# HKUST-Aerial-Robotics/FUEL

Measured on AMD Instinct MI355X. Metric: plan_cycles_per_sec, higher is better.
Workload: dtype u64 bit-planes / u16 (u32 beyond 255 voxels) exact squared distances / f32 ESDF / f64 log-odds and B-spline

## Files before the change

### fuel_amd/csrc/esdf.hip

```cpp
#include <algorithm>
#include <cmath>
#include <vector>

#include "fuelmi_internal.h"

template <int MODE>
__device__ __forceinline__ u64 src_word(const u64* __restrict__ infl, const u64* __restrict__ unk, long w) {
  if (MODE == 0) return infl[w] | unk[w];
  if (MODE == 1) return infl[w];
  return ~infl[w];
}

template <int MODE>
__device__ __forceinline__ int nearest_src(const u64* __restrict__ infl, const u64* __restrict__ unk,
                                           long linebit, int zlo, int zhi, int z) {
  int best = -1;
  {
    long pos = linebit + z, end = linebit + zhi;
    long w = pos >> 6;
    u64 word = src_word<MODE>(infl, unk, w) & (~0ull << (pos & 63));
    while (true) {
      if (word) {
        long c = (w << 6) + __builtin_ctzll(word);
        if (c <= end) best = (int)(c - pos);
// ... 516 lines not shown
  int below, above;
};
template <int NW>
struct LineBits {
  u64 w[NW];
};
template <int MODE, int NW>
__device__ __forceinline__ LineBits<NW> line_load(const u64* __restrict__ infl, const u64* __restrict__ unk, long linebit,
                                                  int z0a, int zlo, int zhi) {
  const long bit0 = linebit + z0a;
  const long w0 = bit0 >> 6;
  const int sh = (int)(bit0 & 63);
  u64 L[NW + 1];
#pragma unroll
  for (int k = 0; k <= NW; ++k) L[k] = src_word<MODE>(infl, unk, w0 + k);
  LineBits<NW> r;
#pragma unroll
  for (int k = 0; k < NW; ++k) {
    const int lo = max(zlo - z0a - 64 * k, 0), hi = min(zhi - z0a - 64 * k, 63);
    const u64 mask = lo <= hi ? bit_range(lo, hi - lo + 1) : 0ull;
    r.w[k] = (sh ? ((L[k] >> sh) | (L[k + 1] << (64 - sh))) : L[k]) & mask;
  }
  return r;
}
template <int NW>
__device__ __forceinline__ u32 line_bits32(const LineBits<NW>& L, int s) {
  const int k = s >> 6, sh = s & 63;
  u64 lo = 0ull, hi = 0ull;
#pragma unroll
  for (int i = 0; i < NW; ++i) {
    if (i == k) lo = L.w[i];
    if (i == k + 1) hi = L.w[i];
  }
  return (u32)(sh ? ((lo >> sh) | (hi << (64 - sh))) : lo);
}
template <int NW>
__device__ __forceinline__ int line_first_from(const LineBits<NW>& L, int s) {
  int pos = -1;
#pragma unroll
  for (int i = NW - 1; i >= 0; --i) {
    u64 m = L.w[i];
    if (64 * i + 63 < s)
      m = 0ull;
    else if (64 * i < s)
      m &= ~0ull << (s - 64 * i);
    if (m) pos = 64 * i + __builtin_ctzll(m);
  }
  return pos;
}
template <int NW>
__device__ __forceinline__ int line_last_below(const LineBits<NW>& L, int s) {
  int pos = -1;
#pragma unroll
  for (int i = 0; i < NW; ++i) {
    u64 m = L.w[i];
    if (64 * i >= s)
      m = 0ull;
    else if (64 * i + 64 > s)
      m &= (1ull << (s - 64 * i)) - 1ull;
    if (m) pos = 64 * i + 63 - __builtin_clzll(m);
  }
  return pos;
}
template <int NW, bool BELOW>
__device__ __forceinline__ RowSrc row_src_line(const LineBits<NW>& L, int z0a, int zc0, int ZC) {
  RowSrc r;
  const int s = zc0 - z0a;
  r.bits = (u64)(line_bits32<NW>(L, s) & (ZC == 32 ? 0xffffffffu : ((1u << ZC) - 1u)));
  const int up = line_first_from<NW>(L, s + ZC);
  r.above = up >= 0 ? z0a + up : -1;
  r.below = -1;
  if (BELOW) {
    const int dn = line_last_below<NW>(L, s);
    r.below = dn >= 0 ? z0a + dn : -1;
  }
  return r;
}

__device__ __forceinline__ u32 bit_fill(u32 v, int zi) {
  u32 r;
  asm("v_bfe_i32 %0, %1, %2, 1" : "=v"(r) : "v"(v), "s"(zi));
  return r;
}
template <int G>
__device__ __forceinline__ u32 zy_fill_pair(u32* prow, u32 bA, u32 bB, u32 d0, int aboveA, int aboveB, int ze, u32 inbox, bool fast) {
  constexpr int ZC = 4 * G;
  const u32 full = ZC == 32 ? 0xffffffffu : ((1u << (ZC & 31)) - 1u);
  if (fast) {
    const bool all_src = bA == inbox && bB == inbox && inbox != 0u;
    const bool no_src = (bA | bB) == 0u && d0 == 0x00ff00ffu && aboveA < 0 && aboveB < 0;
    if (__ballot(!(all_src | no_src)) == 0ull) {
      const u32 v = all_src ? 0u : pk_both(PK_INF);
      const uint4 o = make_uint4(v, v, v, v);
#pragma unroll
      for (int k = 0; k < G; ++k) *reinterpret_cast<uint4*>(prow + 4 * k) = o;
      if (inbox != full) {
        const u32 ib = inbox | (threadIdx.x & 0u);
        for (int zi = 0; zi < ZC; ++zi) prow[zi] &= bit_fill(ib, zi);
      }
      return all_src ? 0u : 0x00ff00ffu;
    }
  }
  const u32 nA = ~bA, nB = ~bB;
  u32 nm[ZC];
  u32 d = d0;
#pragma unroll
  for (int k = 0; k < G; ++k) {
    u32 f[4];
#pragma unroll
    for (int q = 0; q < 4; ++q) {
      const int zi = 4 * k + q;
      nm[zi] = (bit_fill(nA, zi) & 0xffffu) | (bit_fill(nB, zi) & 0xffff0000u);
      d = pk_add(d, 0x00010001u) & nm[zi];
      f[q] = d;
    }
    *reinterpret_cast<uint4*>(prow + 4 * k) = make_uint4(f[0], f[1], f[2], f[3]);
  }
  const u32 d_end = pk_min(d, 0x00ff00ffu);
  d = (aboveA >= 0 ? (u32)min(aboveA - (ze + 1), 255) : 255u) | ((aboveB >= 0 ? (u32)min(aboveB - (ze + 1), 255) : 255u) << 16);
#pragma unroll
  for (int k = G - 1; k >= 0; --k) {
    const uint4 fw = *reinterpret_cast<const uint4*>(prow + 4 * k);
    const u32 f[4] = {fw.x, fw.y, fw.z, fw.w};
    u32 o[4];
#pragma unroll
    for (int q = 3; q >= 0; --q) {
      d = pk_add(d, 0x00010001u) & nm[4 * k + q];
      const u32 t = pk_min(pk_min(f[q], d), 0x00ff00ffu);
      o[q] = pk_mul(t, t);
    }
    *reinterpret_cast<uint4*>(prow + 4 * k) = make_uint4(o[0], o[1], o[2], o[3]);
  }
  if (inbox != full) {
    const u32 ib = inbox | (threadIdx.x & 0u);
    for (int zi = 0; zi < ZC; ++zi) prow[zi] &= bit_fill(ib, zi);
  }
  return d_end;
}
__device__ __forceinline__ u32 pk_below_d0(const RowSrc& A, const RowSrc& B, int zs) {
  return (A.below >= 0 ? (u32)min(zs - 1 - A.below, 255) : 255u) | ((B.below >= 0 ? (u32)min(zs - 1 - B.below, 255) : 255u) << 16);
}

__device__ __noinline__ u32 pk_slow_col(const u32* tile, int ZC, int ylen, int row, int zcol) {
  u32 best = INF32;
  const int rmax = max(row, ylen - 1 - row);
  for (int r = 0; r <= rmax && (u32)(r * r) < best; ++r) {
    const u32 rr = (u32)(r * r);
    if (row - r >= 0) {
      const int q = row - r;
      const u32 v = (tile[(q >> 1) * ZC + zcol] >> (16 * (q & 1))) & 0xffffu;
      if (v < PK_INF) best = min(best, v + rr);
    }
    if (r && row + r < ylen) {
      const int q = row + r;
      const u32 v = (tile[(q >> 1) * ZC + zcol] >> (16 * (q & 1))) & 0xffffu;
      if (v < PK_INF) best = min(best, v + rr);
    }
  }
  return best;
}

template <int G, bool TILE_SLOW = true>
__device__ __forceinline__ void pk_scan8(const unsigned char* tile_b, int p, int gi, int npair, int ylen, bool any_src,
                                         bool sampled, int& n_far, uint4& ra, uint4& rb) {
  constexpr int ZC = 4 * G;
  constexpr int stride = ZC * 4;
  const u32* tile = reinterpret_cast<const u32*>(tile_b);
    const int col = 16 * gi, base = __mul24(p, stride) + col;
    if (!any_src) {
      ra = rb = make_uint4(INF32, INF32, INF32, INF32);
      if (sampled) n_far += __popcll(__ballot(1));
    } else {
      const uint4 v = lds4(tile_b, base);
      u32 b0 = pk_min(v.x, pk_adds(pk_swap(v.x), 0x00010001u)), b1 = pk_min(v.y, pk_adds(pk_swap(v.y), 0x00010001u));
      u32 b2 = pk_min(v.z, pk_adds(pk_swap(v.z), 0x00010001u)), b3 = pk_min(v.w, pk_adds(pk_swap(v.w), 0x00010001u));
      u32 mx = pk_hmax(pk_max(pk_max(b0, b1), pk_max(b2, b3)));
      const int hi_off = __mul24(npair - 1, stride) + col;
      const int jmax = max(p, npair - 1 - p);
      int od = base, ou = base;
      u32 ro2 = 1u, j8 = 8u;
      for (int j = 1; j <= jmax && ro2 < mx; ++j) {
        od = max(od - stride, col);
        ou = min(ou + stride, hi_off);
        const uint4 pd = lds4(tile_b, od), pu = lds4(tile_b, ou);
        const u32 rn2 = ro2 + j8;
        const u32 re2 = (ro2 + rn2 - 2u) >> 1;
        const u32 ke = pk_both(pk_sat16(re2));
        const u32 k1 = pk_sat16(ro2) | (pk_sat16(rn2) << 16), k2 = pk_sat16(rn2) | (pk_sat16(ro2) << 16);
        b0 = pk_min(b0, pk_min(pk_adds(pk_min(pd.x, pu.x), ke), pk_min(pk_adds(pk_swap(pd.x), k1), pk_adds(pk_swap(pu.x), k2))));
        b1 = pk_min(b1, pk_min(pk_adds(pk_min(pd.y, pu.y), ke), pk_min(pk_adds(pk_swap(pd.y), k1), pk_adds(pk_swap(pu.y), k2))));
        b2 = pk_min(b2, pk_min(pk_adds(pk_min(pd.z, pu.z), ke), pk_min(pk_adds(pk_swap(pd.z), k1), pk_adds(pk_swap(pu.z), k2))));
        b3 = pk_min(b3, pk_min(pk_adds(pk_min(pd.w, pu.w), ke), pk_min(pk_adds(pk_swap(pd.w), k1), pk_adds(pk_swap(pu.w), k2))));
        mx = pk_hmax(pk_max(pk_max(b0, b1), pk_max(b2, b3)));
        ro2 = rn2;
        j8 += 8u;
      }
      if (sampled) n_far += __popcll(__ballot(pk_hmin(pk_min(pk_min(b0, b1), pk_min(b2, b3))) > ESDF_FAR_D * ESDF_FAR_D));
      ra = make_uint4(b0 & 0xffffu, b1 & 0xffffu, b2 & 0xffffu, b3 & 0xffffu);
      rb = make_uint4(b0 >> 16, b1 >> 16, b2 >> 16, b3 >> 16);
      if (TILE_SLOW && mx >= PK_INF) {
        const int zc = 4 * gi, rA = 2 * p, rB = 2 * p + 1;
        if (ra.x >= PK_INF) ra.x = pk_slow_col(tile, ZC, ylen, rA, zc);
        if (ra.y >= PK_INF) ra.y = pk_slow_col(tile, ZC, ylen, rA, zc + 1);
        if (ra.z >= PK_INF) ra.z = pk_slow_col(tile, ZC, ylen, rA, zc + 2);
        if (ra.w >= PK_INF) ra.w = pk_slow_col(tile, ZC, ylen, rA, zc + 3);
        if (rB < ylen) {
          if (rb.x >= PK_INF) rb.x = pk_slow_col(tile, ZC, ylen, rB, zc);
          if (rb.y >= PK_INF) rb.y = pk_slow_col(tile, ZC, ylen, rB, zc + 1);
          if (rb.z >= PK_INF) rb.z = pk_slow_col(tile, ZC, ylen, rB, zc + 2);
          if (rb.w >= PK_INF) rb.w = pk_slow_col(tile, ZC, ylen, rB, zc + 3);
        }
      }
    }
}

__device__ __forceinline__ void forward_stat(u32* stat, volatile u32* h_stat_v) {
  if (stat == nullptr || blockIdx.x != 0) return;
  unsigned long long* h_stat = reinterpret_cast<unsigned long long*>(const_cast<u32*>(h_stat_v));
  const u32 e = stat[2 * ESDF_NG] + 1u;
  const unsigned long long tag = (unsigned long long)(e % 65535u + 1u) << 48;
// ... 36 lines not shown
__global__ void __launch_bounds__(1024)
k_esdf_x4(Geo g, Box3 b, const u32* __restrict__ tmp, float* __restrict__ dist, int z0a, int zlen_a, int near,
          u32* stat, volatile u32* h_stat) {
  extern __shared__ __attribute__((aligned(16))) unsigned char smem_raw[];
  forward_stat(stat, h_stat);
  uint4* tile = reinterpret_cast<uint4*>(smem_raw);
  const int xlen = b.hi[0] - b.lo[0] + 1;
  const int ylen = b.hi[1] - b.lo[1] + 1;
  const int ncol = ylen * zlen_a;
  const int seg = threadIdx.x & (SEGS - 1);
  const int row0 = threadIdx.x / SEGS;
  const int rows = blockDim.x / SEGS;
  const int col = blockIdx.x * (4 * SEGS) + seg * 4;
  const bool valid = col < ncol;
  const int yy = valid ? col / zlen_a : 0;
  const int z = z0a + (valid ? col - yy * zlen_a : 0);
  const long coloff = (long)(b.lo[1] + yy) * g.nz + z;
  const uint4 inf4 = make_uint4(INF32, INF32, INF32, INF32);
  const float resf = (float)g.res;
  unsigned char* bm = smem_raw + (size_t)xlen * SEGS * 16;
  u32* cm = reinterpret_cast<u32*>(bm + (size_t)((xlen + 7) >> 3) * SEGS * 16);
#pragma unroll 4
  for (int xi = row0; xi < xlen; xi += rows)
    tile[xi * SEGS + seg] = valid ? *reinterpret_cast<const uint4*>(tmp + (long)(b.lo[0] + xi) * g.nyz + coloff) : inf4;
  if (FAR && (int)threadIdx.x < 4 * SEGS) cm[threadIdx.x] = INF32;
  __syncthreads();
  if (FAR) {
    build_block_minima(smem_raw, bm, cm, SEGS * 16, SEGS, xlen);
    __syncthreads();
  }
  if (!valid) return;
  for (int xi = row0; xi < xlen; xi += rows) {
    const uint4 bb = scan_line4<FAR>(smem_raw, bm, reinterpret_cast<const unsigned char*>(cm), SEGS * 16, xlen, xi, 16 * seg, near);
    x_store4<OUT>(dist + (long)(b.lo[0] + xi) * g.nyz + coloff, z, b.lo[2], b.hi[2], bb, resf);
  }
}

#define PK_NOSRC 0xFFFFu
extern "C" __device__ int __ockl_wgred_or_i32(int a);

template <int G>
__device__ __forceinline__ void pk_scan16(const unsigned char* tA, const unsigned char* tB, int p, int gi, int npair, int want,
                                          u32 (&a)[4], u32 (&c)[4]) {
  constexpr int stride = 16 * G;
  const int col = 16 * gi, base = __mul24(p, stride) + col;
  const uint4 vA = lds4(tA, base), vB = lds4(tB, base);
  const u32 one = 0x00010001u;
  a[0] = pk_min(vA.x, pk_adds(pk_swap(vA.x), one)), a[1] = pk_min(vA.y, pk_adds(pk_swap(vA.y), one));
  a[2] = pk_min(vA.z, pk_adds(pk_swap(vA.z), one)), a[3] = pk_min(vA.w, pk_adds(pk_swap(vA.w), one));
  c[0] = pk_min(vB.x, pk_adds(pk_swap(vB.x), one)), c[1] = pk_min(vB.y, pk_adds(pk_swap(vB.y), one));
  c[2] = pk_min(vB.z, pk_adds(pk_swap(vB.z), one)), c[3] = pk_min(vB.w, pk_adds(pk_swap(vB.w), one));
  const u32 mA = (want & 1) ? 0xffffffffu : 0u, mB = (want & 2) ? 0xffffffffu : 0u;
  u32 mx = pk_hmax(pk_max(pk_max(pk_max(a[0], a[1]), pk_max(a[2], a[3])) & mA, pk_max(pk_max(c[0], c[1]), pk_max(c[2], c[3])) & mB));
  const int hi_off = __mul24(npair - 1, stride) + col;
  const int jmax = max(p, npair - 1 - p);
  int od = base, ou = base;
  u32 ro2 = 1u, j8 = 8u;
  for (int j = 1; j <= jmax && ro2 < mx; ++j) {
    od = max(od - stride, col);
    ou = min(ou + stride, hi_off);
    const uint4 dA = lds4(tA, od), uA = lds4(tA, ou), dB = lds4(tB, od), uB = lds4(tB, ou);
    const u32 rn2 = ro2 + j8;
    const u32 re2 = (ro2 + rn2 - 2u) >> 1;
    const u32 ke = pk_both(pk_sat16(re2));
    const u32 k1 = pk_sat16(ro2) | (pk_sat16(rn2) << 16), k2 = pk_sat16(rn2) | (pk_sat16(ro2) << 16);
#define PK16_STEP(B, D, U) B = pk_min(B, pk_min(pk_adds(pk_min(D, U), ke), pk_min(pk_adds(pk_swap(D), k1), pk_adds(pk_swap(U), k2))))
    PK16_STEP(a[0], dA.x, uA.x);
    PK16_STEP(a[1], dA.y, uA.y);
    PK16_STEP(a[2], dA.z, uA.z);
    PK16_STEP(a[3], dA.w, uA.w);
    PK16_STEP(c[0], dB.x, uB.x);
    PK16_STEP(c[1], dB.y, uB.y);
    PK16_STEP(c[2], dB.z, uB.z);
    PK16_STEP(c[3], dB.w, uB.w);
#undef PK16_STEP
    mx = pk_hmax(pk_max(pk_max(pk_max(a[0], a[1]), pk_max(a[2], a[3])) & mA, pk_max(pk_max(c[0], c[1]), pk_max(c[2], c[3])) & mB));
    ro2 = rn2;
    j8 += 8u;
  }
}

__device__ __forceinline__ size_t pk2_index(int tile, int q, int seg, int npx) { return ((size_t)tile * npx + q) * 8 + seg; }

__device__ __forceinline__ u32 pk2_encode(u32 exact, u32* wide_at, bool in_box) {
  if (exact >= INF32) return PK_NOSRC;
  if (exact < PK_INF) return exact;
  if (in_box) *wide_at = exact;
  return PK_INF;
}


template <int MODE, int G, int NW>
__device__ __forceinline__ void zy_pk2_body(const Geo& g, const Box3& b, const u64* __restrict__ infl, const u64* __restrict__ unk,
                                            uint4* __restrict__ tmp16, u32* __restrict__ wide, int z0a, int seg0, int tile0, int tstride, int gsh,
                                            int off, int npx, int q, int fastrow, u32* __restrict__ stat, u32* __restrict__ src_flag, u32 serial,
                                            unsigned long long* stamp, unsigned char* smem_raw) {
  constexpr int ZC = 4 * G;
  const int xA = b.lo[0] + 2 * q, xB = min(xA + 1, b.hi[0]);
  const int zc0 = z0a + 4 * seg0;
  const int ylen = b.hi[1] - b.lo[1] + 1;
  const int npair = (ylen + 1) >> 1;
  const int T = blockDim.x, TH = T >> 1;
  const int half = (int)threadIdx.x >= TH ? 1 : 0;
  const int x = half ? xB : xA;
  unsigned char* tA = smem_raw;
  unsigned char* tB = smem_raw + (size_t)npair * ZC * 4;
  u32* tile = reinterpret_cast<u32*>(half ? tB : tA);
  const int zs = max(zc0, b.lo[2]), ze = min(zc0 + ZC - 1, b.hi[2]);
  const u32 inbox = zs <= ze ? (u32)bit_range(zs - zc0, ze - zs + 1) : 0u;
  bool has_src = false;
  for (int p = (int)threadIdx.x - half * TH; p < npair; p += TH) {
    const int yA = 2 * p, yB = min(2 * p + 1, ylen - 1);
    const long lbA = (long)x * g.nyz + (long)(b.lo[1] + yA) * g.nz;
    const long lbB = (long)x * g.nyz + (long)(b.lo[1] + yB) * g.nz;
    RowSrc A, B;
    A.bits = B.bits = 0ull;
    A.below = A.above = B.below = B.above = -1;
    if (zs <= ze) {
      const LineBits<NW> LA = line_load<MODE, NW>(infl, unk, lbA, z0a, b.lo[2], b.hi[2]);
      const LineBits<NW> LB = line_load<MODE, NW>(infl, unk, lbB, z0a, b.lo[2], b.hi[2]);
      A = row_src_line<NW, true>(LA, z0a, zc0, ZC);
      B = row_src_line<NW, true>(LB, z0a, zc0, ZC);
    }
    has_src |= (A.bits | B.bits) != 0ull || A.below >= 0 || A.above >= 0 || B.below >= 0 || B.above >= 0;
    (void)zy_fill_pair<G>(tile + p * ZC, (u32)A.bits, (u32)B.bits, pk_below_d0(A, B, zs), A.above, B.above, ze, inbox, (fastrow & 1) != 0);
  }
  if (stamp && threadIdx.x == 0) stamp[1] = wall_clock64();
  const int want = __ockl_wgred_or_i32(has_src ? (1 << half) : 0);
  if (stamp && threadIdx.x == 0) stamp[2] = wall_clock64();
  if (want && threadIdx.x == 0) *src_flag = serial;
  const int total = npair * G;
  const bool sampA = stat != nullptr && ((xA & 15) == 0 || q == 0);
  const bool sampB = stat != nullptr && xB != xA && (xB & 15) == 0;
  int n_farA = 0, n_farB = 0;
  for (int o = threadIdx.x; o < total; o += T) {
    const int p = o / G, gi = o - p * G;
    u32 a[4], c[4];
    if (want) {
      pk_scan16<G>(tA, tB, p, gi, npair, want, a, c);
    } else {
      a[0] = a[1] = a[2] = a[3] = c[0] = c[1] = c[2] = c[3] = pk_both(PK_INF);
    }
    if (sampA) n_farA += __popcll(__ballot(!(want & 1) || pk_hmin(pk_min(pk_min(a[0], a[1]), pk_min(a[2], a[3]))) > ESDF_FAR_D * ESDF_FAR_D));
    if (sampB) n_farB += __popcll(__ballot(!(want & 2) || pk_hmin(pk_min(pk_min(c[0], c[1]), pk_min(c[2], c[3]))) > ESDF_FAR_D * ESDF_FAR_D));
    uint4 r0, r1;
    const u32 mxa = pk_hmax(pk_max(pk_max(a[0], a[1]), pk_max(a[2], a[3]))), mxc = pk_hmax(pk_max(pk_max(c[0], c[1]), pk_max(c[2], c[3])));
    if (max(mxa, mxc) < PK_INF) {
      r0 = make_uint4(__builtin_amdgcn_perm(c[0], a[0], 0x05040100u), __builtin_amdgcn_perm(c[1], a[1], 0x05040100u),
                      __builtin_amdgcn_perm(c[2], a[2], 0x05040100u), __builtin_amdgcn_perm(c[3], a[3], 0x05040100u));
      r1 = make_uint4(__builtin_amdgcn_perm(c[0], a[0], 0x07060302u), __builtin_amdgcn_perm(c[1], a[1], 0x07060302u),
                      __builtin_amdgcn_perm(c[2], a[2], 0x07060302u), __builtin_amdgcn_perm(c[3], a[3], 0x07060302u));
    } else {
      const int zc = 4 * gi, rA = 2 * p, rB = min(2 * p + 1, ylen - 1);
      u32 w0[4], w1[4];
#pragma unroll
      for (int k = 0; k < 4; ++k) {
        const int z = zc0 + zc + k;
        const bool in_box = z >= b.lo[2] && z <= b.hi[2];
        u32 e[4];
        e[0] = a[k] & 0xffffu, e[1] = a[k] >> 16, e[2] = c[k] & 0xffffu, e[3] = c[k] >> 16;
#pragma unroll
        for (int v = 0; v < 4; ++v) {
          const bool slabB = v >= 2;
          const int row = (v & 1) ? rB : rA;
          if (!((want >> (slabB ? 1 : 0)) & 1))
            e[v] = in_box ? PK_NOSRC : 0u;
          else if (e[v] >= PK_INF) {
            const u32 ex = pk_slow_col(reinterpret_cast<const u32*>(slabB ? tB : tA), ZC, ylen, row, zc + k);
            u32* wat = wide + (long)(slabB ? xB : xA) * g.nyz + (long)(b.lo[1] + row) * g.nz + z;
            e[v] = pk2_encode(ex, wat, in_box);
          }
        }
        w0[k] = e[0] | (e[2] << 16), w1[k] = e[1] | (e[3] << 16);
      }
      r0 = make_uint4(w0[0], w0[1], w0[2], w0[3]);
      r1 = make_uint4(w1[0], w1[1], w1[2], w1[3]);
    }
    {
      const int y = 2 * p, ry1 = (8 >> gsh) - 1;
      store16(tmp16 + pk2_index(tile0 + (y >> (3 - gsh)) * tstride, q, ((y & ry1) << gsh) + off + gi, npx), r0);
    }
    if (2 * p + 1 < ylen) {
      const int y = 2 * p + 1, ry1 = (8 >> gsh) - 1;
      store16(tmp16 + pk2_index(tile0 + (y >> (3 - gsh)) * tstride, q, ((y & ry1) << gsh) + off + gi, npx), r1);
    }
  }
  if (stamp && threadIdx.x == 0) stamp[3] = wall_clock64();
  if ((sampA | sampB) && (threadIdx.x & 63) == 0) {
    if (sampA) {
      u32* sg = stat + 2 * ((xA >> 4) & (ESDF_NG - 1));
      atomicAdd(sg, (u32)n_farA);
      if (threadIdx.x == 0) atomicAdd(sg + 1, (u32)total);
    }
    if (sampB) {
      u32* sg = stat + 2 * ((xB >> 4) & (ESDF_NG - 1));
      atomicAdd(sg, (u32)n_farB);
      if (threadIdx.x == 0) atomicAdd(sg + 1, (u32)total);
    }
  }
}

template <int MODE, int GMAX, int NW>
__global__ void __launch_bounds__(1024)
k_esdf_zy_pk2(Geo g, Box3 b, const u64* __restrict__ infl, const u64* __restrict__ unk, uint4* __restrict__ tmp16,
              u32* __restrict__ wide, Pk2ZChunks ch, int z0a, int npx, int fastrow, u32* __restrict__ stat,
              u32* __restrict__ src_flag, u32 serial, unsigned long long* __restrict__ dbg) {
  extern __shared__ __attribute__((aligned(16))) unsigned char smem_raw[];
  const int nzc = ch.n;
  const int xcd = blockIdx.x & 7, slot = blockIdx.x >> 3;
  const int q = xcd + 8 * (slot / nzc);
  if (q >= npx) return;
// ... 35 lines not shown

template <int OUT>
__global__ void __launch_bounds__(512)
k_esdf_x_pk2(Geo g, Box3 b, const uint4* __restrict__ tmp16, const u32* __restrict__ wide, float* __restrict__ dist, Pk2Chunks ch,
             int z0a, int full8, u32* stat, volatile u32* h_stat, const u32* __restrict__ src_flag, u32 serial,
             unsigned long long* __restrict__ dbg) {
  constexpr int SEGS = 8;
  extern __shared__ __attribute__((aligned(16))) unsigned char smem_raw[];
  forward_stat(stat, h_stat);
  uint4* tile = reinterpret_cast<uint4*>(smem_raw);
  const int xlen = b.hi[0] - b.lo[0] + 1;
  const int ylen = b.hi[1] - b.lo[1] + 1;
  const int npx = (xlen + 1) >> 1;
  const int T = blockDim.x;
  const int total = npx * SEGS;
  const float resf = (float)g.res;
  unsigned long long* stamp = dbg ? dbg + 8 * (size_t)blockIdx.x : nullptr;
  if (stamp && threadIdx.x == 0) stamp[0] = wall_clock64();
  int gw = 8, gsh = 3, y0, seg0, t;
  if ((int)blockIdx.x < full8) {
    const int xcd = blockIdx.x & 7, slot = blockIdx.x >> 3;
    y0 = xcd + 8 * (slot / ch.n8);
    if (y0 >= ylen) return;
    const int c8 = slot % ch.n8;
    seg0 = 8 * c8;
    t = y0 * ch.n8 + c8;
  } else {
    t = (int)blockIdx.x - full8 + ylen * ch.n8;
    int c = ch.n8;
    while (c + 1 < ch.n && t >= ch.tile0[c + 1]) ++c;
    gw = ch.g[c], gsh = gw == 4 ? 2 : (gw == 2 ? 1 : 0);
    y0 = (t - ch.tile0[c]) * (8 >> gsh);
    seg0 = ch.seg0[c];
  }
  const bool any_src = *src_flag == serial;
  if (any_src) {
    const uint4* src = tmp16 + pk2_index(t, 0, 0, npx);
#pragma unroll 4
    for (int o = threadIdx.x; o < total; o += T) tile[o] = src[o];
  }
  if (stamp && threadIdx.x == 0) stamp[1] = wall_clock64();
  __syncthreads();
  if (stamp && threadIdx.x == 0) stamp[2] = wall_clock64();
  int n_far = 0;
  for (int o = threadIdx.x; o < total; o += T) {
    const int p = o >> 3, seg = o & 7;
    const int yy = y0 + (seg >> gsh);
    if (yy >= ylen) continue;
    uint4 ra, rb;
    pk_scan8<SEGS, false>(smem_raw, p, seg, npx, xlen, any_src, false, n_far, ra, rb);
    const int z = z0a + 4 * (seg0 + (seg & (gw - 1)));
    const long coloff = (long)(b.lo[1] + yy) * g.nz + z;
    if (any_src && max(max4(ra.x, ra.y, ra.z, ra.w), max4(rb.x, rb.y, rb.z, rb.w)) >= PK_INF) {
      u32* pa = &ra.x;
      u32* pb = &rb.x;
      const u32* wc = wide + (long)b.lo[0] * g.nyz + coloff;
      for (int k = 0; k < 4; ++k) {
        if (pa[k] >= PK_INF) pa[k] = x_slow_col16(reinterpret_cast<const u32*>(smem_raw), 4 * seg + k, wc + k, g.nyz, xlen, 2 * p);
        if (2 * p + 1 < xlen && pb[k] >= PK_INF)
          pb[k] = x_slow_col16(reinterpret_cast<const u32*>(smem_raw), 4 * seg + k, wc + k, g.nyz, xlen, 2 * p + 1);
      }
    }
    float* dst = dist + (long)(b.lo[0] + 2 * p) * g.nyz + coloff;
    x_store4<OUT>(dst, z, b.lo[2], b.hi[2], ra, resf);
    if (2 * p + 1 < xlen) x_store4<OUT>(dst + g.nyz, z, b.lo[2], b.hi[2], rb, resf);
  }
  if (stamp && threadIdx.x == 0) stamp[3] = wall_clock64();
}


static hipError_t lds_attr_once(const void* fn, int bytes) {
  static std::mutex mu;
  static std::vector<std::pair<const void*, int>> done;
  int dev = 0;
  (void)hipGetDevice(&dev);
  std::lock_guard<std::mutex> lk(mu);
  for (const auto& d : done)
    if (d.first == fn && d.second == dev) return hipSuccess;
  const hipError_t e = hipFuncSetAttribute(fn, hipFuncAttributeMaxDynamicSharedMemorySize, bytes);
  if (e == hipSuccess) done.push_back({fn, dev});
  return e;
}

static int pass_timing_report(fuelmi_map* m, unsigned long long* dbg, int grid, const char* what) {
  HIPCHK(hipStreamSynchronize(m->stream));
  std::vector<unsigned long long> d((size_t)grid * 8);
  HIPCHK(hipMemcpy(d.data(), dbg, d.size() * sizeof(unsigned long long), hipMemcpyDeviceToHost));
  HIPCHK(hipFree(dbg));
  unsigned long long t0 = ~0ull, t1 = 0;
  double ph[3] = {0, 0, 0}, life = 0;
  int n = 0;
  for (int w = 0; w < grid; ++w) {
    const unsigned long long* r = &d[(size_t)w * 8];
    if (!r[0] || !r[3]) continue;
    t0 = std::min(t0, r[0]), t1 = std::max(t1, r[3]);
    ph[0] += (double)(r[1] - r[0]), ph[1] += (double)(r[2] - r[1]), ph[2] += (double)(r[3] - r[2]), life += (double)(r[3] - r[0]);
    ++n;
  }
  int alive = 0, early = 0;
  const unsigned long long mid = t0 + (t1 - t0) / 2;
  for (int w = 0; w < grid; ++w) {
    const unsigned long long* r = &d[(size_t)w * 8];
    if (!r[0] || !r[3]) continue;
    if (r[0] <= mid && r[3] >= mid) ++alive;
    if (r[0] - t0 < 100) ++early;
  }
  std::vector<double> st, en;
  for (int w = 0; w < grid; ++w) {
    const unsigned long long* r = &d[(size_t)w * 8];
    if (!r[0] || !r[3]) continue;
    st.push_back((double)(r[0] - t0) / 100.0), en.push_back((double)(r[3] - t0) / 100.0);
  }
  std::sort(st.begin(), st.end());
  std::sort(en.begin(), en.end());
  int peak = 0;
  {
    size_t i = 0, j = 0;
    int cur = 0;
    while (i < st.size()) {
      if (st[i] <= en[j]) ++cur, ++i, peak = std::max(peak, cur);
      else --cur, ++j;
    }
  }
  {
    std::vector<std::pair<double, int>> lv;
    for (int w = 0; w < grid; ++w) {
      const unsigned long long* r = &d[(size_t)w * 8];
      if (!r[0] || !r[3]) continue;
      lv.push_back({(double)(r[3] - r[0]) / 100.0, w});
    }
    std::sort(lv.begin(), lv.end());
    const size_t k0 = lv.size() - std::max<size_t>(1, lv.size() / 10);
    double f = 0, bb = 0, sc = 0, lf = 0;
    for (size_t k = k0; k < lv.size(); ++k) {
      const unsigned long long* r = &d[(size_t)lv[k].second * 8];
      f += (double)(r[1] - r[0]), bb += (double)(r[2] - r[1]), sc += (double)(r[3] - r[2]), lf += lv[k].first;
    }
    const double nn = (double)(lv.size() - k0) * 100.0;
    std::fprintf(stderr, "[slowest tenth: fill %.2f barrier %.2f scan %.2f life %.2f us; slowest blocks:", f / nn, bb / nn, sc / nn, lf * 100.0 / nn);
    for (size_t k = lv.size() - std::min<size_t>(8, lv.size()); k < lv.size(); ++k) std::fprintf(stderr, " %d(%.1f)", lv[k].second, lv[k].first);
    std::fprintf(stderr, "]\n");
  }
  auto pct = [](const std::vector<double>& v, double f) { return v.empty() ? 0.0 : v[std::min(v.size() - 1, (size_t)(f * (double)v.size()))]; };
  std::fprintf(stderr, "[%s: %d workgroups, span %.2f us; per workgroup: fill %.2f barrier %.2f scan %.2f life %.2f us; "
               "alive at mid-span %d (peak %d), started in the first us %d; starts 25/50/75/100 %%: %.1f %.1f %.1f %.1f us, ends 25/50/75: %.1f %.1f %.1f\n",
               what, n, (double)(t1 - t0) / 100.0, ph[0] / n / 100.0,
               ph[1] / n / 100.0, ph[2] / n / 100.0, life / n / 100.0, alive, peak, early, pct(st, 0.25), pct(st, 0.5), pct(st, 0.75),
               pct(st, 1.0), pct(en, 0.25), pct(en, 0.5), pct(en, 0.75));
  return FUELMI_OK;
}


static bool pk2_chunks(int ylen, int nseg, int gz_max, Pk2Chunks* xs, Pk2ZChunks* zs) {
  *xs = Pk2Chunks{};
  *zs = Pk2ZChunks{};
  const int n8 = nseg >> 3;
  int n = 0, nz = 0, seg = 0, tile = ylen * n8;
  auto add_z = [&](int seg_lo, int gw, int gsh, int tile0, int tstride) {
    const int gz = std::min(gw, gz_max);
    for (int o = 0; o < gw; o += gz) {
      if (nz == PK2_MAXZCH) return false;
      zs->seg0[nz] = (short)(seg_lo + o), zs->g[nz] = (signed char)gz, zs->gsh[nz] = (signed char)gsh, zs->off[nz] = (signed char)o;
      zs->tile0[nz] = tile0, zs->tstride[nz] = tstride;
      ++nz;
    }
    return true;
  };
  for (int c = 0; c < n8; ++c, ++n, seg += 8) {
    if (n == PK2_MAXCH) return false;
    xs->seg0[n] = (short)seg, xs->g[n] = 8, xs->tile0[n] = 0;
    if (!add_z(seg, 8, 3, c, n8)) return false;
  }
  xs->n8 = n8;
  while (seg < nseg) {
    int gw = 4;
    while (gw > nseg - seg) gw >>= 1;
    const int gsh = gw == 4 ? 2 : (gw == 2 ? 1 : 0);
    if (n == PK2_MAXCH) return false;
    xs->seg0[n] = (short)seg, xs->g[n] = (short)gw, xs->tile0[n] = tile;
    if (!add_z(seg, gw, gsh, tile, 1)) return false;
    tile += (ylen + 8 / gw - 1) / (8 / gw);
    seg += gw;
    ++n;
  }
  xs->n = n;
  zs->n = nz;
  for (int k = n; k <= PK2_MAXCH; ++k) xs->tile0[k] = tile;
  for (int k = n; k < PK2_MAXCH; ++k) xs->g[k] = 1;
  if (n8 == n) xs->tile0[n8] = tile;
  return true;
}

size_t esdf_handover_bytes(int nx, int ny, int nz) {
  if (nz % 4 != 0) return 0;
  const size_t ntiles = ((size_t)ny * (size_t)((nz + 7) / 4 + 1) + 7) / 8 + PK2_MAXCH + 1;
  return ntiles * (size_t)(((nx + 1) / 2 + 63) / 64) * 64 * 128;
}

struct EsdfLaunch {
  int kernel = 0, targ[3] = {0, 0, 0};
  int grid = 0, block = 0, lds = 0;
  int ZC = 0, nzc = 0, z0a = 0;
  int aux = 0;
};
struct EsdfPlan {
  int n = 0;
  int family = 0;
  EsdfLaunch l[4];
  Pk2Chunks ch;
  Pk2ZChunks zch;
};

static int esdf_plan(const int dims[3], const Box3& b, int family, bool optimistic, bool signed_dist, size_t handover,
                     EsdfPlan* p) {
  *p = EsdfPlan{};
  const int xlen = b.hi[0] - b.lo[0] + 1, ylen = b.hi[1] - b.lo[1] + 1, zlen = b.hi[2] - b.lo[2] + 1;
  const int z0a = b.lo[2] & ~3, zlen_a = (b.hi[2] | 3) - z0a + 1;
  const int npx = (xlen + 1) >> 1, npair = (ylen + 1) >> 1;
  const bool z4 = dims[2] % 4 == 0;
  const int g_max = (size_t)npair * 4 * 32 > 52 * 1024 ? 2 : 4;
  const size_t pk2_lds = (size_t)npair * g_max * 32;
  const bool pk2 = z4 && zlen <= 255 && handover > 0 && (size_t)npx * 128 <= 150 * 1024 && pk2_lds <= 160 * 1024 - 64 &&
                   pk2_chunks(ylen, zlen_a >> 2, g_max, &p->ch, &p->zch) &&
                   (size_t)p->ch.tile0[p->ch.n] * npx * 128 <= handover;
  const bool vec4 = z4 && (size_t)xlen * 64 <= 150 * 1024;

  auto pass = [&](int fam, int mode, EsdfLaunch* L, int* ran) {
    const int out = mode == 2;
    EsdfLaunch& zy = L[0];
    EsdfLaunch& x = L[1];
    if (fam == FUELMI_ESDF_PLAIN && pk2) {
      zy = {FUELMI_ESDF_K_ZY_PK2, {mode, g_max, zlen_a > 128 ? 4 : 2}, ((npx + 7) / 8) * 8 * p->zch.n,
            2 * std::min(256, std::max(64, ((npair / 2 + 63) / 64) * 64)), (int)pk2_lds, 0, p->zch.n, z0a, npx};
      const int x_lds = npx * 8 * 16;
      const int full8 = ((ylen + 7) / 8) * 8 * p->ch.n8;
      x = {FUELMI_ESDF_K_X_PK2, {out, 0, 0}, full8 + (p->ch.tile0[p->ch.n] - ylen * p->ch.n8), x_lds > 32 * 1024 ? 512 : 256,
           x_lds, 0, p->ch.n, z0a, full8};
      *ran = FUELMI_ESDF_PLAIN;
      return FUELMI_OK;
    }
    const bool far = fam == FUELMI_ESDF_FAR;
    *ran = far ? FUELMI_ESDF_FAR : FUELMI_ESDF_PLAIN32;
    if (vec4) {
      const int budget = std::min(std::max(32 * 1024, ylen * 4 * 20), 80 * 1024);
      int zc_max = std::max(4, (budget / (4 * ylen)) & ~3);
      zc_max = std::min(zc_max, std::min(zlen_a, 64));
      int nzc = (zlen_a + zc_max - 1) / zc_max;
      const int ZC = (((zlen_a + nzc - 1) / nzc) + 3) & ~3;
      nzc = (zlen_a + ZC - 1) / ZC;
      auto zy_lds = [&](bool f) { return (size_t)(f ? ylen + ((ylen + 7) >> 3) + 1 : ylen) * ZC * sizeof(u32); };
      const bool zy_far = far && zy_lds(true) <= 160 * 1024;
      if (zy_lds(zy_far) > 160 * 1024) {
        fuelmi_set_error("ESDF y-line of %d voxels does not fit the LDS tile", ylen);
        return FUELMI_ELIMIT;
      }
      zy = {FUELMI_ESDF_K_ZY4, {mode, zy_far, 0}, ((xlen + 7) / 8) * 8 * nzc, 512, (int)zy_lds(zy_far), ZC, nzc, z0a, 0};
      const int segs = (size_t)xlen * 128 > 150 * 1024 ? 4 : 8;
      auto x_lds = [&](bool f) { return (size_t)(f ? xlen + ((xlen + 7) >> 3) + 1 : xlen) * segs * 4 * sizeof(u32); };
      const bool x_far = far && x_lds(true) <= 160 * 1024;
      x = {FUELMI_ESDF_K_X4, {out, segs, x_far}, (ylen * zlen_a + 4 * segs - 1) / (4 * segs), 1024, (int)x_lds(x_far), 0, 0,
           z0a, zlen_a};
      return FUELMI_OK;
    }
    const int zc_max = std::min(std::min(std::max(1, (16 * 1024) / (2 * ylen)), zlen), 256);
    const int nzc = (zlen + zc_max - 1) / zc_max;
    const int ZC = (zlen + nzc - 1) / nzc;
    const size_t lds = (size_t)ylen * ZC * sizeof(unsigned short);
    if (lds > 160 * 1024) {
      fuelmi_set_error("ESDF y-line of %d voxels does not fit the LDS tile", ylen);
      return FUELMI_ELIMIT;
    }
    zy = {FUELMI_ESDF_K_ZY, {mode, 0, 0}, xlen * nzc, 256, (int)lds, ZC, nzc, 0, 0};
    const int S = (size_t)xlen * 32 * 4 <= 64 * 1024 ? 32 : ((size_t)xlen * 16 * 4 <= 128 * 1024 ? 16 : ((size_t)xlen * 8 * 4 <= 128 * 1024 ? 8 : 0));
    if (!S) {
      fuelmi_set_error("ESDF x-line of %d voxels does not fit the LDS tile", xlen);
      return FUELMI_ELIMIT;
    }
    x = {FUELMI_ESDF_K_X, {S, out, 0}, (ylen * zlen + S - 1) / S, 256, xlen * S * (int)sizeof(u32), 0, 0, 0, 0};
    return FUELMI_OK;
  };

  int rc = pass(family, optimistic ? 1 : 0, &p->l[0], &p->family);
  if (rc) return rc;
  p->n = 2;
  if (signed_dist) {
    int ran;
    rc = pass(family == FUELMI_ESDF_FAR ? FUELMI_ESDF_PLAIN : family, 2, &p->l[2], &ran);
    if (rc) return rc;
    p->n = 4;
  }
  return FUELMI_OK;
}

static volatile u32* esdf_stat_host(fuelmi_map* m) { return m->h_esdf_stat; }
static u32 pk2_next_serial(fuelmi_map* m) {
  if (++m->esdf_serial == 0u) m->esdf_serial = 1u;
  return m->esdf_serial;
}
static u32* pk2_src_flag(fuelmi_map* m) { return m->esdf_stat + 2 * ESDF_NG + 2; }

static bool esdf_use_far(fuelmi_map* m, const Box3& b) {
  const volatile unsigned long long* h = reinterpret_cast<const volatile unsigned long long*>(esdf_stat_host(m));
  const int g_lo = b.lo[0] >> 4, g_n = std::min((b.hi[0] >> 4) - g_lo + 1, ESDF_NG);
  for (int gi = 0; gi < g_n; ++gi) {
    const int g = (g_lo + gi) & (ESDF_NG - 1);
    const unsigned long long v = h[g];
    const unsigned short tag = (unsigned short)(v >> 48);
    if (tag != 0 && tag != m->far_tag[g]) {
      m->far_tag[g] = tag;
      m->far_hist[g][0] = (u32)(v & 0xffffffu);
      m->far_hist[g][1] = (u32)((v >> 24) & 0xffffffu);
    }
  }
  unsigned long long nf = 0, nt = 0;
  for (int g = b.lo[0] >> 4; g <= (b.hi[0] >> 4); ++g) nf += m->far_hist[g & (ESDF_NG - 1)][0], nt += m->far_hist[g & (ESDF_NG - 1)][1];
  if (nt != 0) m->far_last = 2 * nf > nt;
  static const bool dbg = getenv("FUELMI_ESDF_DEBUG") != nullptr;
  if (dbg) std::fprintf(stderr, "[fuelmi] esdf regime: far %llu of %llu sampled outputs -> %s kernels\n", nf, nt,
                        m->far_last ? "far-field" : "plain");
  return m->far_last;
}


template <class K, class... A>
static int esdf_launch(fuelmi_map* m, K kern, const EsdfLaunch& L, int lds_cap, A... args) {
  if (L.lds > 64 * 1024) HIPCHK(lds_attr_once(reinterpret_cast<const void*>(kern), lds_cap));
  STAGE_LAUNCH(m, kern, L.grid, L.block, L.lds, args...);
  HIPCHK(hipGetLastError());
  return FUELMI_OK;
}

template <class F>
static int timed_launch(fuelmi_map* m, const EsdfLaunch& L, F launch) {
  static const bool timing = getenv("FUELMI_ZY_TIMING") != nullptr;
  unsigned long long* dbg = nullptr;
  if (timing) {
    HIPCHK(hipMalloc(reinterpret_cast<void**>(&dbg), (size_t)L.grid * 8 * sizeof(unsigned long long)));
    HIPCHK(hipMemsetAsync(dbg, 0, (size_t)L.grid * 8 * sizeof(unsigned long long), m->stream));
  }
  const int rc = launch(dbg);
  if (rc != FUELMI_OK || !timing) return rc;
  char what[96];
  if (L.kernel == FUELMI_ESDF_K_ZY_PK2)
    std::snprintf(what, sizeof what, "zy2-timing] GMAX %d chunks %d threads %d lds %d", L.targ[1], L.nzc, L.block, L.lds);
  else
    std::snprintf(what, sizeof what, "x2-timing] threads %d lds %d", L.block, L.lds);
  return pass_timing_report(m, dbg, L.grid, what);
}

template <int MODE>
static int launch_zy(fuelmi_map* m, const Box3& b, const EsdfPlan& p, const EsdfLaunch& L) {
  const Geo& g = m->g;
  const u64* infl = m->infl_bits.p;
  const u64* unk = m->unk_bits.p;
  u32* stat = MODE == 2 ? nullptr : m->esdf_stat;
  if (L.kernel == FUELMI_ESDF_K_ZY) return esdf_launch(m, &k_esdf_zy<MODE>, L, 160 * 1024, g, b, infl, unk, m->esdf_tmp, L.ZC, L.nzc);
  if (L.kernel == FUELMI_ESDF_K_ZY4) {
    auto go = [&](auto kern) {
      return esdf_launch(m, kern, L, 160 * 1024, g, b, infl, unk, m->esdf_tmp, L.ZC, L.nzc, L.z0a, ESDF_NEAR | (ZY_FASTROW << 8), stat);
    };
    if constexpr (MODE != 2)
      if (L.targ[1]) return go(&k_esdf_zy4<MODE, true>);
    return go(&k_esdf_zy4<MODE, false>);
  }
  const u32 serial = pk2_next_serial(m);
  return timed_launch(m, L, [&](unsigned long long* dbg) {
    auto go = [&](auto kern) {
      return esdf_launch(m, kern, L, 160 * 1024, g, b, infl, unk, reinterpret_cast<uint4*>(m->esdf_tmp16), m->esdf_tmp,
                         p.zch, L.z0a, L.aux, ZY_FASTROW, stat, pk2_src_flag(m), serial, dbg);
    };
    const bool g4 = L.targ[1] == 4, nw4 = L.targ[2] == 4;
    return g4 ? (nw4 ? go(&k_esdf_zy_pk2<MODE, 4, 4>) : go(&k_esdf_zy_pk2<MODE, 4, 2>))
              : (nw4 ? go(&k_esdf_zy_pk2<MODE, 2, 4>) : go(&k_esdf_zy_pk2<MODE, 2, 2>));
  });
}

template <int OUT>
static int launch_x(fuelmi_map* m, const Box3& b, const EsdfPlan& p, const EsdfLaunch& L) {
  const Geo& g = m->g;
  u32* stat = OUT == 0 ? m->esdf_stat : nullptr;
  if (L.kernel == FUELMI_ESDF_K_X) {
    auto go = [&](auto kern) { return esdf_launch(m, kern, L, 160 * 1024, g, b, (const u32*)m->esdf_tmp, m->dist); };
    return L.targ[0] == 32 ? go(&k_esdf_x<32, OUT>) : (L.targ[0] == 16 ? go(&k_esdf_x<16, OUT>) : go(&k_esdf_x<8, OUT>));
  }
  if (L.kernel == FUELMI_ESDF_K_X4) {
    auto go = [&](auto kern) {
      return esdf_launch(m, kern, L, 160 * 1024, g, b, (const u32*)m->esdf_tmp, m->dist, L.z0a, L.aux, ESDF_NEAR, stat,
                         esdf_stat_host(m));
    };
    const bool segs8 = L.targ[1] == 8;
    if constexpr (OUT == 0)
      if (L.targ[2]) return segs8 ? go(&k_esdf_x4<OUT, 8, true>) : go(&k_esdf_x4<OUT, 4, true>);
    return segs8 ? go(&k_esdf_x4<OUT, 8, false>) : go(&k_esdf_x4<OUT, 4, false>);
  }
  return timed_launch(m, L, [&](unsigned long long* dbg) {
    return esdf_launch(m, &k_esdf_x_pk2<OUT>, L, 150 * 1024, g, b, reinterpret_cast<const uint4*>(m->esdf_tmp16),
                       (const u32*)m->esdf_tmp, m->dist, p.ch, L.z0a, L.aux, stat, esdf_stat_host(m),
                       (const u32*)pk2_src_flag(m), m->esdf_serial, dbg);
  });
}

static bool esdf_is_zy(const EsdfLaunch& L) { return L.kernel <= FUELMI_ESDF_K_ZY_PK2; }


int esdf_update(fuelmi_map* m) {
  const Box3& b = m->local_bound;
  const int fam = m->esdf_family_pin >= 0 ? m->esdf_family_pin : (esdf_use_far(m, b) ? FUELMI_ESDF_FAR : FUELMI_ESDF_PLAIN);
  const int dims[3] = {m->g.nx, m->g.ny, m->g.nz};
  EsdfPlan p;
  int rc = esdf_plan(dims, b, fam, m->cfg.optimistic != 0, m->cfg.signed_dist != 0, m->esdf_tmp16_bytes, &p);
  if (rc) return rc;
  m->esdf_family_last = p.family;
  for (int i = 0; i < p.n && rc == FUELMI_OK; ++i) {
    const EsdfLaunch& L = p.l[i];
    StageScope sc(m, esdf_is_zy(L) ? FUELMI_K_ESDF_ZY : FUELMI_K_ESDF_X, nullptr, true);
    if (esdf_is_zy(L))
      rc = L.targ[0] == 0 ? launch_zy<0>(m, b, p, L) : (L.targ[0] == 1 ? launch_zy<1>(m, b, p, L) : launch_zy<2>(m, b, p, L));
    else
      rc = (L.kernel == FUELMI_ESDF_K_X ? L.targ[1] : L.targ[0]) == 0 ? launch_x<0>(m, b, p, L) : launch_x<1>(m, b, p, L);
  }
  return rc;
}

extern "C" int fuelmi_map_esdf_plan(const int dims[3], const int lo[3], const int hi[3], int family, int flags,
                                    int out[FUELMI_ESDF_PLAN_INTS]) {
  ARGCHK(dims && lo && hi && out && family >= FUELMI_ESDF_PLAIN && family <= FUELMI_ESDF_PLAIN32);
  Box3 b;
  for (int i = 0; i < 3; ++i) {
    ARGCHK(dims[i] > 0 && 0 <= lo[i] && lo[i] <= hi[i] && hi[i] < dims[i]);
    b.lo[i] = lo[i], b.hi[i] = hi[i];
  }
  EsdfPlan p;
  const int rc = esdf_plan(dims, b, family, (flags & FUELMI_ESDF_PLAN_OPTIMISTIC) != 0, (flags & FUELMI_ESDF_PLAN_SIGNED) != 0,
                           esdf_handover_bytes(dims[0], dims[1], dims[2]), &p);
  if (rc) return rc;
  for (int k = 0; k < FUELMI_ESDF_PLAN_INTS; ++k) out[k] = 0;
  out[0] = p.n, out[1] = p.family;
  for (int i = 0; i < p.n; ++i) {
    const EsdfLaunch& L = p.l[i];
    const int v[10] = {L.kernel, L.targ[0], L.targ[1], L.targ[2], L.grid, L.block, L.lds, L.ZC, L.nzc, L.z0a};
    for (int k = 0; k < 10; ++k) out[2 + 10 * i + k] = v[k];
  }
  return FUELMI_OK;
}

extern "C" int fuelmi_map_set_esdf_family(fuelmi_map* m, int family) {
  ARGCHK(m && family >= FUELMI_ESDF_AUTO && family <= FUELMI_ESDF_PLAIN32);
  m->esdf_family_pin = family;
  return FUELMI_OK;
}
extern "C" int fuelmi_map_last_esdf_family(const fuelmi_map* m) {
  ARGCHK(m);
  return m->esdf_family_last;
}
```

Measured before the change: 11040.

## Compact non-constant zy rows into a shared-memory work list before sweeping

The zy pk2 fill now treats each (slab, row-pair) as one flat task. Constant rows (all-source or no-source) are written directly per thread. The remaining rows park their parameters in LDS and are appended to a work list through a wave ballot and atomic, then swept in a second compacted pass, replacing the old wave-uniform ballot fast path. The goal is to cut divergence and idle lanes, since one non-constant lane previously forced the whole wave into the full sweep. The cost is extra LDS for the list, an added barrier and atomic, and a tighter LDS budget for choosing pk2.

```diff
diff --git a/fuel_amd/csrc/esdf.hip b/fuel_amd/csrc/esdf.hip
--- a/fuel_amd/csrc/esdf.hip
+++ b/fuel_amd/csrc/esdf.hip
@@ -622,25 +622,34 @@
   asm("v_bfe_i32 %0, %1, %2, 1" : "=v"(r) : "v"(v), "s"(zi));
   return r;
 }
+__device__ __forceinline__ bool zy_row_is_const(u32 bA, u32 bB, u32 d0, u32 dbk, u32 inbox, bool& all_src) {
+  all_src = bA == inbox && bB == inbox && inbox != 0u;
+  const bool no_src = (bA | bB) == 0u && d0 == 0x00ff00ffu && dbk == 0x00ff00ffu;
+  return all_src | no_src;
+}
+__device__ __forceinline__ u32 pk_above_dbk(int aboveA, int aboveB, int ze) {
+  return (aboveA >= 0 ? (u32)min(aboveA - (ze + 1), 255) : 255u) | ((aboveB >= 0 ? (u32)min(aboveB - (ze + 1), 255) : 255u) << 16);
+}
 template <int G>
-__device__ __forceinline__ u32 zy_fill_pair(u32* prow, u32 bA, u32 bB, u32 d0, int aboveA, int aboveB, int ze, u32 inbox, bool fast) {
+__device__ __forceinline__ void zy_mask_pair(u32* prow, u32 inbox) {
+  constexpr int ZC = 4 * G;
+  const u32 ib = inbox | (threadIdx.x & 0u);
+  for (int zi = 0; zi < ZC; ++zi) prow[zi] &= bit_fill(ib, zi);
+}
+template <int G>
+__device__ __forceinline__ void zy_const_pair(u32* prow, bool all_src, u32 inbox) {
   constexpr int ZC = 4 * G;
   const u32 full = ZC == 32 ? 0xffffffffu : ((1u << (ZC & 31)) - 1u);
-  if (fast) {
-    const bool all_src = bA == inbox && bB == inbox && inbox != 0u;
-    const bool no_src = (bA | bB) == 0u && d0 == 0x00ff00ffu && aboveA < 0 && aboveB < 0;
-    if (__ballot(!(all_src | no_src)) == 0ull) {
-      const u32 v = all_src ? 0u : pk_both(PK_INF);
-      const uint4 o = make_uint4(v, v, v, v);
+  const u32 v = all_src ? 0u : pk_both(PK_INF);
+  const uint4 o = make_uint4(v, v, v, v);
 #pragma unroll
-      for (int k = 0; k < G; ++k) *reinterpret_cast<uint4*>(prow + 4 * k) = o;
-      if (inbox != full) {
-        const u32 ib = inbox | (threadIdx.x & 0u);
-        for (int zi = 0; zi < ZC; ++zi) prow[zi] &= bit_fill(ib, zi);
-      }
-      return all_src ? 0u : 0x00ff00ffu;
-    }
-  }
+  for (int k = 0; k < G; ++k) *reinterpret_cast<uint4*>(prow + 4 * k) = o;
+  if (inbox != full) zy_mask_pair<G>(prow, inbox);
+}
+template <int G>
+__device__ __forceinline__ void zy_sweep_pair(u32* prow, u32 bA, u32 bB, u32 d0, u32 dbk, u32 inbox) {
+  constexpr int ZC = 4 * G;
+  const u32 full = ZC == 32 ? 0xffffffffu : ((1u << (ZC & 31)) - 1u);
   const u32 nA = ~bA, nB = ~bB;
   u32 nm[ZC];
   u32 d = d0;
@@ -656,8 +665,7 @@
     }
     *reinterpret_cast<uint4*>(prow + 4 * k) = make_uint4(f[0], f[1], f[2], f[3]);
   }
-  const u32 d_end = pk_min(d, 0x00ff00ffu);
-  d = (aboveA >= 0 ? (u32)min(aboveA - (ze + 1), 255) : 255u) | ((aboveB >= 0 ? (u32)min(aboveB - (ze + 1), 255) : 255u) << 16);
+  d = dbk;
 #pragma unroll
   for (int k = G - 1; k >= 0; --k) {
     const uint4 fw = *reinterpret_cast<const uint4*>(prow + 4 * k);
@@ -671,11 +679,7 @@
     }
     *reinterpret_cast<uint4*>(prow + 4 * k) = make_uint4(o[0], o[1], o[2], o[3]);
   }
-  if (inbox != full) {
-    const u32 ib = inbox | (threadIdx.x & 0u);
-    for (int zi = 0; zi < ZC; ++zi) prow[zi] &= bit_fill(ib, zi);
-  }
-  return d_end;
+  if (inbox != full) zy_mask_pair<G>(prow, inbox);
 }
 __device__ __forceinline__ u32 pk_below_d0(const RowSrc& A, const RowSrc& B, int zs) {
   return (A.below >= 0 ? (u32)min(zs - 1 - A.below, 255) : 255u) | ((B.below >= 0 ? (u32)min(zs - 1 - B.below, 255) : 255u) << 16);
@@ -878,6 +882,8 @@
 
 __device__ __forceinline__ size_t pk2_index(int tile, int q, int seg, int npx) { return ((size_t)tile * npx + q) * 8 + seg; }
 
+static inline size_t pk2_list_bytes(int npair) { return ((size_t)4 + (size_t)4 * npair + 15) & ~(size_t)15; }
+
 __device__ __forceinline__ u32 pk2_encode(u32 exact, u32* wide_at, bool in_box) {
   if (exact >= INF32) return PK_NOSRC;
   if (exact < PK_INF) return exact;
@@ -896,33 +902,64 @@
   const int zc0 = z0a + 4 * seg0;
   const int ylen = b.hi[1] - b.lo[1] + 1;
   const int npair = (ylen + 1) >> 1;
-  const int T = blockDim.x, TH = T >> 1;
-  const int half = (int)threadIdx.x >= TH ? 1 : 0;
-  const int x = half ? xB : xA;
+  const int T = blockDim.x;
   unsigned char* tA = smem_raw;
   unsigned char* tB = smem_raw + (size_t)npair * ZC * 4;
-  u32* tile = reinterpret_cast<u32*>(half ? tB : tA);
+  u32* rows = reinterpret_cast<u32*>(smem_raw);
+  u32* s_nsweep = reinterpret_cast<u32*>(smem_raw + (size_t)2 * npair * ZC * 4);
+  unsigned short* s_sweep = reinterpret_cast<unsigned short*>(s_nsweep + 1);
   const int zs = max(zc0, b.lo[2]), ze = min(zc0 + ZC - 1, b.hi[2]);
   const u32 inbox = zs <= ze ? (u32)bit_range(zs - zc0, ze - zs + 1) : 0u;
-  bool has_src = false;
-  for (int p = (int)threadIdx.x - half * TH; p < npair; p += TH) {
-    const int yA = 2 * p, yB = min(2 * p + 1, ylen - 1);
-    const long lbA = (long)x * g.nyz + (long)(b.lo[1] + yA) * g.nz;
-    const long lbB = (long)x * g.nyz + (long)(b.lo[1] + yB) * g.nz;
-    RowSrc A, B;
-    A.bits = B.bits = 0ull;
-    A.below = A.above = B.below = B.above = -1;
-    if (zs <= ze) {
-      const LineBits<NW> LA = line_load<MODE, NW>(infl, unk, lbA, z0a, b.lo[2], b.hi[2]);
-      const LineBits<NW> LB = line_load<MODE, NW>(infl, unk, lbB, z0a, b.lo[2], b.hi[2]);
-      A = row_src_line<NW, true>(LA, z0a, zc0, ZC);
-      B = row_src_line<NW, true>(LB, z0a, zc0, ZC);
-    }
-    has_src |= (A.bits | B.bits) != 0ull || A.below >= 0 || A.above >= 0 || B.below >= 0 || B.above >= 0;
-    (void)zy_fill_pair<G>(tile + p * ZC, (u32)A.bits, (u32)B.bits, pk_below_d0(A, B, zs), A.above, B.above, ze, inbox, (fastrow & 1) != 0);
-  }
-  if (stamp && threadIdx.x == 0) stamp[1] = wall_clock64();
-  const int want = __ockl_wgred_or_i32(has_src ? (1 << half) : 0);
+  if (threadIdx.x == 0) *s_nsweep = 0u;
+  __syncthreads();
+  const int ntask = 2 * npair;
+  int has_src = 0;
+  for (int t0 = 0; t0 < ntask; t0 += T) {
+    const int t = t0 + (int)threadIdx.x;
+    bool park = false;
+    if (t < ntask) {
+      const int slab = t >= npair ? 1 : 0, p = t - slab * npair;
+      const int x = slab ? xB : xA;
+      const int yA = 2 * p, yB = min(2 * p + 1, ylen - 1);
+      const long lbA = (long)x * g.nyz + (long)(b.lo[1] + yA) * g.nz;
+      const long lbB = (long)x * g.nyz + (long)(b.lo[1] + yB) * g.nz;
+      RowSrc A, B;
+      A.bits = B.bits = 0ull;
+      A.below = A.above = B.below = B.above = -1;
+      if (zs <= ze) {
+        const LineBits<NW> LA = line_load<MODE, NW>(infl, unk, lbA, z0a, b.lo[2], b.hi[2]);
+        const LineBits<NW> LB = line_load<MODE, NW>(infl, unk, lbB, z0a, b.lo[2], b.hi[2]);
+        A = row_src_line<NW, true>(LA, z0a, zc0, ZC);
+        B = row_src_line<NW, true>(LB, z0a, zc0, ZC);
+      }
+      if ((A.bits | B.bits) != 0ull || A.below >= 0 || A.above >= 0 || B.below >= 0 || B.above >= 0) has_src |= 1 << slab;
+      const u32 bA = (u32)A.bits, bB = (u32)B.bits, d0 = pk_below_d0(A, B, zs), dbk = pk_above_dbk(A.above, B.above, ze);
+      u32* prow = rows + (size_t)t * ZC;
+      bool all_src;
+      if ((fastrow & 1) != 0 && zy_row_is_const(bA, bB, d0, dbk, inbox, all_src)) {
+        zy_const_pair<G>(prow, all_src, inbox);
+      } else {
+        *reinterpret_cast<uint4*>(prow) = make_uint4(bA, bB, d0, dbk);
+        park = true;
+      }
+    }
+    const u64 pm = __ballot(park);
+    if (pm != 0ull) {
+      u32 base = 0u;
+      if ((threadIdx.x & 63) == 0) base = atomicAdd(s_nsweep, (u32)__popcll(pm));
+      base = (u32)__builtin_amdgcn_readfirstlane((int)base);
+      if (park) s_sweep[base + __builtin_amdgcn_mbcnt_hi((u32)(pm >> 32), __builtin_amdgcn_mbcnt_lo((u32)pm, 0u))] = (unsigned short)t;
+    }
+  }
+  __syncthreads();
+  const int nsweep = (int)*s_nsweep;
+  for (int i = threadIdx.x; i < nsweep; i += T) {
+    u32* prow = rows + (size_t)s_sweep[i] * ZC;
+    const uint4 r = *reinterpret_cast<const uint4*>(prow);
+    zy_sweep_pair<G>(prow, r.x, r.y, r.z, r.w, inbox);
+  }
+  if (stamp && threadIdx.x == 0) stamp[1] = wall_clock64(), stamp[4] = (unsigned long long)nsweep;
+  const int want = __ockl_wgred_or_i32(has_src);
   if (stamp && threadIdx.x == 0) stamp[2] = wall_clock64();
   if (want && threadIdx.x == 0) *src_flag = serial;
   const int total = npair * G;
@@ -1124,7 +1161,7 @@
   return e;
 }
 
-static int pass_timing_report(fuelmi_map* m, unsigned long long* dbg, int grid, const char* what) {
+static int pass_timing_report(fuelmi_map* m, unsigned long long* dbg, int grid, const char* what, int ntask) {
   HIPCHK(hipStreamSynchronize(m->stream));
   std::vector<unsigned long long> d((size_t)grid * 8);
   HIPCHK(hipMemcpy(d.data(), dbg, d.size() * sizeof(unsigned long long), hipMemcpyDeviceToHost));
@@ -1183,6 +1220,16 @@
     for (size_t k = lv.size() - std::min<size_t>(8, lv.size()); k < lv.size(); ++k) std::fprintf(stderr, " %d(%.1f)", lv[k].second, lv[k].first);
     std::fprintf(stderr, "]\n");
   }
+  if (ntask > 0) {
+    unsigned long long rows = 0, trips = 0, mx = 0;
+    for (int w = 0; w < grid; ++w) {
+      const unsigned long long* r = &d[(size_t)w * 8];
+      if (!r[0] || !r[3]) continue;
+      rows += r[4], trips += (r[4] + 63) / 64, mx = std::max(mx, r[4]);
+    }
+    std::fprintf(stderr, "[fill: %d tasks = %d prologue wave-trips per workgroup; sweep rows %.1f (max %llu) = %.2f sweep wave-trips per workgroup, %llu in all]\n",
+                 ntask, (ntask + 63) / 64, (double)rows / std::max(n, 1), mx, (double)trips / std::max(n, 1), trips);
+  }
   auto pct = [](const std::vector<double>& v, double f) { return v.empty() ? 0.0 : v[std::min(v.size() - 1, (size_t)(f * (double)v.size()))]; };
   std::fprintf(stderr, "[%s: %d workgroups, span %.2f us; per workgroup: fill %.2f barrier %.2f scan %.2f life %.2f us; "
                "alive at mid-span %d (peak %d), started in the first us %d; starts 25/50/75/100 %%: %.1f %.1f %.1f %.1f us, ends 25/50/75: %.1f %.1f %.1f\n",
@@ -1262,7 +1309,8 @@
   const bool z4 = dims[2] % 4 == 0;
   const int g_max = (size_t)npair * 4 * 32 > 52 * 1024 ? 2 : 4;
   const size_t pk2_lds = (size_t)npair * g_max * 32;
-  const bool pk2 = z4 && zlen <= 255 && handover > 0 && (size_t)npx * 128 <= 150 * 1024 && pk2_lds <= 160 * 1024 - 64 &&
+  const bool pk2 = z4 && zlen <= 255 && handover > 0 && (size_t)npx * 128 <= 150 * 1024 &&
+                   pk2_lds + pk2_list_bytes(npair) <= 160 * 1024 - 64 &&
                    pk2_chunks(ylen, zlen_a >> 2, g_max, &p->ch, &p->zch) &&
                    (size_t)p->ch.tile0[p->ch.n] * npx * 128 <= handover;
   const bool vec4 = z4 && (size_t)xlen * 64 <= 150 * 1024;
@@ -1373,7 +1421,7 @@
 }
 
 template <class F>
-static int timed_launch(fuelmi_map* m, const EsdfLaunch& L, F launch) {
+static int timed_launch(fuelmi_map* m, const EsdfLaunch& L, F launch, int ntask = 0) {
   static const bool timing = getenv("FUELMI_ZY_TIMING") != nullptr;
   unsigned long long* dbg = nullptr;
   if (timing) {
@@ -1387,7 +1435,7 @@
     std::snprintf(what, sizeof what, "zy2-timing] GMAX %d chunks %d threads %d lds %d", L.targ[1], L.nzc, L.block, L.lds);
   else
     std::snprintf(what, sizeof what, "x2-timing] threads %d lds %d", L.block, L.lds);
-  return pass_timing_report(m, dbg, L.grid, what);
+  return pass_timing_report(m, dbg, L.grid, what, ntask);
 }
 
 template <int MODE>
@@ -1406,15 +1454,17 @@
     return go(&k_esdf_zy4<MODE, false>);
   }
   const u32 serial = pk2_next_serial(m);
-  return timed_launch(m, L, [&](unsigned long long* dbg) {
+  EsdfLaunch LL = L;
+  LL.lds += (int)pk2_list_bytes((b.hi[1] - b.lo[1] + 2) >> 1);
+  return timed_launch(m, LL, [&](unsigned long long* dbg) {
     auto go = [&](auto kern) {
-      return esdf_launch(m, kern, L, 160 * 1024, g, b, infl, unk, reinterpret_cast<uint4*>(m->esdf_tmp16), m->esdf_tmp,
+      return esdf_launch(m, kern, LL, 160 * 1024, g, b, infl, unk, reinterpret_cast<uint4*>(m->esdf_tmp16), m->esdf_tmp,
                          p.zch, L.z0a, L.aux, ZY_FASTROW, stat, pk2_src_flag(m), serial, dbg);
     };
     const bool g4 = L.targ[1] == 4, nw4 = L.targ[2] == 4;
     return g4 ? (nw4 ? go(&k_esdf_zy_pk2<MODE, 4, 4>) : go(&k_esdf_zy_pk2<MODE, 4, 2>))
               : (nw4 ? go(&k_esdf_zy_pk2<MODE, 2, 4>) : go(&k_esdf_zy_pk2<MODE, 2, 2>));
-  });
+  }, 2 * ((b.hi[1] - b.lo[1] + 2) >> 1));
 }
 
 template <int OUT>
```

Result: no change. 10960 (-0.7%).
